# bobocode/lmono

Measured on AMD Instinct MI355X. Metric: KITTI HDL-64 scans/sec (scanRegistration + laserOdometry), higher is better.
Workload: dtype f32 features / f64 solve

## Files before the change

lmono_amd/csrc/frontend.hip:

```cpp
#include "batch.hpp"
#include "ring_decide.hpp"

namespace lmono {

__device__ __forceinline__ int ring_of(float angle, int n_lines, bool &discard)
{
    int id = 0;
    discard = false;
    if (n_lines == 16) {
        id = (int)((double)((angle + 15.0f) / 2.0f) + 0.5);
        if (id > n_lines - 1 || id < 0) discard = true;
    } else if (n_lines == 32) {
        id = (int)(((double)angle + 92.0 / 3.0) * 3.0 / 4.0);
        if (id > n_lines - 1 || id < 0) discard = true;
    } else {
        if ((double)angle >= -8.83)
            id = (int)((double)(2.0f - angle) * 3.0 + 0.5);
        else
            id = n_lines / 2 + (int)((-8.83 - (double)angle) * 2.0 + 0.5);
        if ((double)angle > 2.0 || (double)angle < -24.33 || id > 50 || id < 0) discard = true;
    }
    return id;
}

__device__ __forceinline__ bool point_valid(const float4 &p, float mr2)
{
    return isfinite(p.x) & isfinite(p.y) & isfinite(p.z) & !(p.x * p.x + p.y * p.y + p.z * p.z < mr2);
}

constexpr int kRtT = 256, kRtW = kRtT / 64;
constexpr int kRtSeg = 1024;
constexpr int kRtTile = kRtSeg * kRtW;

__device__ __forceinline__ int ring_scan_points(const BatchView &b, int s, int64_t off)
{
    const int n = (int)(b.off[s + 1] - off);
    return b.n_limit > 0 && b.n_limit < n ? b.n_limit : n;
}

__global__ __launch_bounds__(256) void k_ring_ends(BatchView b)
{
    const int s = b.scan0 + blockIdx.x;
    const int64_t off = b.off[s];
    const int n = ring_scan_points(b, s, off);
    const float4 *in = b.in + off;
    const int tid = threadIdx.x, lane = tid & 63;
    __shared__ int s_first;
    if (tid == 0) s_first = INT_MAX;
    __syncthreads();
    const float mr2 = b.min_range * b.min_range;
    for (int c0 = 0; c0 < n; c0 += 256) {
        const int i = c0 + tid;
        int lf = (i < n && point_valid(in[i], mr2)) ? i : INT_MAX;
        lf = wave_min_i(lf);
        if (lane == 0 && lf != INT_MAX) atomicMin(&s_first, lf);
        __syncthreads();
        const int f = s_first;
        __syncthreads();
        if (f != INT_MAX) break;
    }
    if (s_first == INT_MAX) {
        int *rb = b.ring_begin + s * 65;
        if (tid < 65) rb[tid] = 0;
        if (tid == 0) { b.n_cloud[s] = 0; b.scan_ends[s * 2] = -1; b.scan_ends[s * 2 + 1] = -1; b.scan_half[s] = INT_MAX; }
        return;
    }
    if (tid == 0) {
        const float4 p0 = in[s_first];
        b.scan_ori[s * 4] = (float)(-det_atan2((double)p0.y, (double)p0.x));
        float ux, uy;
        ring_start_dir(p0.x, p0.y, ux, uy);
        b.scan_ori[s * 4 + 2] = ux; b.scan_ori[s * 4 + 3] = uy;
        b.scan_ends[s * 2] = s_first; b.scan_ends[s * 2 + 1] = -1;
        b.scan_half[s] = INT_MAX;
    }
}

__global__ __launch_bounds__(kRtT) void k_ring_tag(BatchView b)
{
    const int s = b.scan0 + blockIdx.y;
    const int64_t off = b.off[s];
    const int n = ring_scan_points(b, s, off);
    const int t0 = blockIdx.x * kRtTile;
    if (t0 >= n || b.scan_ends[s * 2] < 0) return;
    const float4 *in = b.in + off;
    const int tid = threadIdx.x, lane = tid & 63, wave = tid >> 6;
    __shared__ int s_hist[kRtW][64];
    s_hist[wave][lane] = 0;
    __syncthreads();
    const float mr2 = b.min_range * b.min_range;
    const float startOri = b.scan_ori[s * 4];
    const float ux = b.scan_ori[s * 4 + 2], uy = b.scan_ori[s * 4 + 3];
    const int n_lines = b.n_lines;
    const RingMap map = ring_map(n_lines);
    int lh = INT_MAX, ll = -1;
    const int c_lo = t0 + wave * kRtSeg, c_hi = min(c_lo + kRtSeg, n);
    float4 nx[4];
#pragma unroll
    for (int q = 0; q < 4; q++) nx[q] = in[min(c_lo + 64 * q + lane, n - 1)];
    for (int r0 = c_lo; r0 < c_hi; r0 += 256) {
        float4 pq[4];
#pragma unroll
        for (int q = 0; q < 4; q++) pq[q] = nx[q];
#pragma unroll
        for (int q = 0; q < 4; q++) nx[q] = in[min(r0 + 256 + 64 * q + lane, n - 1)];
#pragma unroll
        for (int q = 0; q < 4; q++) {
            const int i = r0 + 64 * q + lane;
            const float4 p = pq[q];
            int id = -1;
            if ((i < c_hi) & point_valid(p, mr2)) {
                ll = i;
                const float q2 = p.x * p.x + p.y * p.y;
                bool past_half;
                if (!ring_half_fast(p.x, p.y, p.z, q2, __frsqrt_rn(q2) , map, ux, uy, id, past_half)) {
                    bool discard;
                    const float angle = (float)(det_atan((double)p.z / sqrt((double)(p.x * p.x + p.y * p.y))) * 180.0 / LM_PI);
                    const int r = ring_of(angle, n_lines, discard);
                    id = -1; past_half = false;
                    if (!discard) {
                        id = r;
                        float o1 = (float)(-det_atan2((double)p.y, (double)p.x));
                        if ((double)o1 < (double)startOri - LM_PI / 2.0) o1 = (float)((double)o1 + 2.0 * LM_PI);
                        else if ((double)o1 > (double)startOri + LM_PI * 3.0 / 2.0) o1 = (float)((double)o1 - 2.0 * LM_PI);
                        past_half = (double)(o1 - startOri) > LM_PI;
                    }
                }
                if (past_half) lh = min(lh, i);
            }
            if (i < c_hi) b.ring_tmp[off + i] = (int8_t)id;
            unsigned long long rem = __ballot(id >= 0);
            while (rem) {
                const int src = __ffsll((long long)rem) - 1;
                const int k = __shfl(id, src);
                const unsigned long long m = __ballot(id == k);
                if (lane == src) s_hist[wave][k] += __popcll(m);
                rem &= ~m;
            }
        }
    }
    lh = wave_min_i(lh); ll = wave_max_i(ll);
    if (lane == 0 && lh != INT_MAX) atomicMin(&b.scan_half[s], lh);
    if (lane == 0 && ll >= 0) atomicMax(&b.scan_ends[s * 2 + 1], ll);
    __syncthreads();
    if (c_lo < n) b.seg_hist[((size_t)(off >> 10) + (size_t)s + (size_t)(c_lo >> 10)) * 64 + lane] = s_hist[wave][lane];
}

__global__ __launch_bounds__(64) void k_ring_offsets(BatchView b)
{
    const int s = b.scan0 + blockIdx.x;
    if (b.scan_ends[s * 2] < 0) return;
    const int64_t off = b.off[s];
    const int n = ring_scan_points(b, s, off);
    const int nseg = (n + kRtSeg - 1) / kRtSeg, r = threadIdx.x;
// ... 184 lines not shown
            if (mh == 0u) break;
            const unsigned long long who = __ballot(ch == mh);
            unsigned int lo;
            if ((who & (who - 1ull)) == 0ull) lo = (unsigned int)__builtin_amdgcn_readlane((int)cl, __ffsll((long long)who) - 1);
            else lo = wave_max_u32_uniform(ch == mh ? cl : 0u);
            const int pind = (int)(lo >> 8), lf = (int)(lo & 15u), lb = (int)((lo >> 4) & 15u);
            largest++;
            if (largest > 20) break;
            if (lane == 0) { sel_sh[j * 20 + largest - 1] = rbeg + pind; label[pind] = largest <= 2 ? 2 : 1; }
            if (lane <= lf + lb) picked[pind - lb + lane] = 1;
            if ((unsigned int)((int)(cl >> 8) - (pind - lb)) <= (unsigned int)(lb + lf)) ch = 0u;
            {
                const int a = pind - lb - sp - lane;
                const int m0 = (a + 63) >> 6;
                if (m0 >= 0 && m0 < M && 64 * m0 <= a + lb + lf) dead |= 1u << m0;
            }
        }
    }
    while (!compact) {
        const unsigned int live = big & ~dead;
        unsigned int bh = 0u, bl = 0u;
#pragma unroll
        for (int m = 0; m < M; m++) {
            const unsigned int h = kh[m] & (unsigned int)((int)(live << (31 - m)) >> 31);
            const bool t = h >= bh;
            bh = t ? h : bh; bl = t ? kl[m] : bl;
        }
        const unsigned int mh = wave_max_u32_uniform(bh);
        if (mh == 0u) break;
        const unsigned long long who = __ballot(bh == mh);
        unsigned int lo;
        if ((who & (who - 1ull)) == 0ull) lo = (unsigned int)__builtin_amdgcn_readlane((int)bl, __ffsll((long long)who) - 1);
        else lo = wave_max_u32_uniform(bh == mh ? bl : 0u);
        const int pind = (int)(lo >> 8), lf = (int)(lo & 15u), lb = (int)((lo >> 4) & 15u);
        largest++;
        if (largest > 20) break;
        if (lane == 0) { sel_sh[j * 20 + largest - 1] = rbeg + pind; label[pind] = largest <= 2 ? 2 : 1; }
        if (lane <= lf + lb) picked[pind - lb + lane] = 1;
        {
            const int a = pind - lb - sp - lane;
            const int m0 = (a + 63) >> 6;
            if (m0 >= 0 && m0 < M && 64 * m0 <= a + lb + lf) dead |= 1u << m0;
        }
    }
    if (lane == 0) sel_sh_n[j] = largest > 20 ? 20 : largest;
    int smallest = 0;
    while (true) {
        const unsigned int live = small & ~dead;
        unsigned int bh = ~0u, bl = ~0u;
#pragma unroll
        for (int m = 0; m < M; m++) {
            const unsigned int h = kh[m] | ~(unsigned int)((int)(live << (31 - m)) >> 31);
            const bool t = h < bh;
            bh = t ? h : bh; bl = t ? kl[m] : bl;
        }
        const unsigned int mh = wave_min_u32_uniform(bh);
        if (mh == ~0u) break;
        const unsigned long long who = __ballot(bh == mh);
        unsigned int lo;
        if ((who & (who - 1ull)) == 0ull) lo = (unsigned int)__builtin_amdgcn_readlane((int)bl, __ffsll((long long)who) - 1);
        else lo = wave_min_u32_uniform(bh == mh ? bl : ~0u);
        const int pind = (int)(lo >> 8), lf = (int)(lo & 15u), lb = (int)((lo >> 4) & 15u);
        if (lane == 0) { label[pind] = -1; sel_fl[j * 4 + smallest] = rbeg + pind; }
        smallest++;
        if (smallest >= 4) break;
        if (lane <= lf + lb) picked[pind - lb + lane] = 1;
        {
            const int a = pind - lb - sp - lane;
            const int m0 = (a + 63) >> 6;
            if (m0 >= 0 && m0 < M && 64 * m0 <= a + lb + lf) dead |= 1u << m0;
        }
    }
    if (lane == 0) sel_fl_n[j] = smallest;
}

__device__ __forceinline__ int uni(int v) { return __builtin_amdgcn_readfirstlane(v); }
__device__ __forceinline__ long long uni64(long long v)
{
    const unsigned int lo = (unsigned int)__builtin_amdgcn_readfirstlane((int)(unsigned int)v), hi = (unsigned int)__builtin_amdgcn_readfirstlane((int)(unsigned int)((unsigned long long)v >> 32));
    return (long long)(((unsigned long long)hi << 32) | lo);
}
template <typename T> __device__ __forceinline__ T *uni_ptr(T *p)
{
    typedef __attribute__((address_space(1))) T GT;
    return (T *)(GT *)uni64((long long)p);
}

__host__ __device__ constexpr int sel_slice_bytes(int cap) { return 2 * cap; }

__device__ __forceinline__ void select_ring(BatchView &b, int r, int s, int lane, unsigned char *smem_w, int cap, bool may_defer, unsigned int *scratch)
{
    r = uni(r); s = uni(s);
    const int64_t off = uni64(b.off[s]);
    const int *rb = b.ring_begin + s * 65;
    const int rbeg = uni(rb[r]), rend = uni(rb[r + 1]), len = rend - rbeg;
    const int S = rbeg + 5, E = rend - 6;
    int *sel_sh = uni_ptr(b.sel_sharp + (size_t)((s * 64 + r) * kSectors) * 20);
    int *sel_sh_n = uni_ptr(b.sel_sharp_n + (s * 64 + r) * kSectors);
    int *sel_fl = uni_ptr(b.sel_flat + (size_t)((s * 64 + r) * kSectors) * 4);
    int *sel_fl_n = uni_ptr(b.sel_flat_n + (s * 64 + r) * kSectors);
    if (E - S < 6 || len > kRingCap) {
        if (lane < kSectors) { sel_sh_n[lane] = 0; sel_fl_n[lane] = 0; }
        if (lane == 0 && len > kRingCap) atomicOr(&b.status[s], kStatusRingOverflow);
        for (int i = lane; i < len; i += 64) b.label[off + rbeg + i] = 0;
        return;
    }
    if (len > cap) {
        if (may_defer && lane == 0) b.sel_todo[1 + atomicAdd(&b.sel_todo[0], 1)] = (s << 6) | r;
        return;
    }
    unsigned char *picked = smem_w;
    signed char *label = uni_ptr((signed char *)(b.label + off + rbeg));
    const float *curv = uni_ptr(b.curv + off + rbeg);
    const int span = E - S;
    unsigned long long *gap = (unsigned long long *)(picked + cap);
    for (int i0 = 0; i0 < len + 64; i0 += 64) {
        const int i = i0 + lane;
        unsigned char g = 0;
        if (i < len) { picked[i] = 0; label[i] = 0; g = b.gap[off + rbeg + i]; }
        const unsigned long long mk = __ballot(g != 0);
        if (lane == 0) gap[i0 >> 6] = mk;
    }
    __builtin_amdgcn_wave_barrier();
    for (int j = 0; j < kSectors; j++) {
        const int sp = 5 + span * j / 6;
        const int ep = 5 + span * (j + 1) / 6 - 1;
        const int slen = ep - sp + 1;
        if (slen <= 5 * 64) select_sector<5>(lane, j, sp, slen, rbeg, curv, picked, label, gap, sel_sh, sel_sh_n, sel_fl, sel_fl_n, scratch);
        else if (slen <= 6 * 64) select_sector<6>(lane, j, sp, slen, rbeg, curv, picked, label, gap, sel_sh, sel_sh_n, sel_fl, sel_fl_n, scratch);
        else select_sector<kSelMaxPerLane>(lane, j, sp, slen, rbeg, curv, picked, label, gap, sel_sh, sel_sh_n, sel_fl, sel_fl_n, scratch);
    }
}

constexpr int kSelSmallCap = 2304, kSelBigGrid = 128;

__global__ __launch_bounds__(256, 8) void k_select(BatchView b, int cap, int from_list)
{
    const int lane = threadIdx.x & 63, wave = __builtin_amdgcn_readfirstlane((int)(threadIdx.x >> 6));
    extern __shared__ __align__(16) unsigned char smem[];
    unsigned char *smem_w = smem + wave * sel_slice_bytes(cap);
    unsigned int *scratch = (unsigned int *)(smem + 4 * sel_slice_bytes(cap) + wave * kSelScratch);
    if (!from_list) {
        select_ring(b, blockIdx.x * 4 + wave, b.scan0 + blockIdx.y, lane, smem_w, cap, true, scratch);
    } else {
        const int n_todo = b.sel_todo[0];
        for (int k = blockIdx.x * 4 + wave; k < n_todo; k += gridDim.x * 4) {
            const int e = b.sel_todo[1 + k];
            select_ring(b, e & 63, e >> 6, lane, smem_w, cap, false, scratch);
        }
    }
}

constexpr int kVoxBucketSegsBig = 1024;
constexpr int kVoxSmallSlots = 9, kVoxSmallBits = 10;
constexpr int kVoxBigSlots = kRingCap / 256, kVoxBigBits = 12;
constexpr int kVoxBigGrid = 512;
template <int kSlots, int kBits, bool kSmall>
struct VoxCfg {
    static constexpr int kSegCap = kSmall ? 256 * kSlots : kVoxBucketSegsBig;
    static constexpr int kHistBytes = (1 << kBits) * 4 > kSegCap * 2 ? (1 << kBits) * 4 : kSegCap * 2;
    static constexpr int kKeyBytes = kSmall ? kSegCap * 4 + kSegCap * 2 + kSegCap * 2 + kHistBytes : kRingCap * 8;
    static constexpr int kLds = kKeyBytes + 1024 + kSlots * 4 * 8 + kSlots * 4 * 4;
};
constexpr int kVoxLdsSmall = VoxCfg<kVoxSmallSlots, kVoxSmallBits, true>::kLds;
constexpr int kVoxLdsBig = VoxCfg<kVoxBigSlots, kVoxBigBits, false>::kLds;
static_assert(2 * kVoxBucketSegsBig * 8 + (1 << kVoxBigBits) * 4 <= kRingCap * 8, "bucket sort scratch must fit the key region");
#ifdef LMONO_VOX_PROF
#define VT(i) { if (blockIdx.x == 20 && blockIdx.y == 3 && threadIdx.x == 0) vt[i] = clock64(); }
#else
#define VT(i)
#endif

__device__ __forceinline__ float wave_min_f(float v)
{
#pragma unroll
    for (int o = 32; o > 0; o >>= 1) v = fminf(v, __shfl_xor(v, o));
    return v;
}
__device__ __forceinline__ float wave_max_f(float v)
{
#pragma unroll
    for (int o = 32; o > 0; o >>= 1) v = fmaxf(v, __shfl_xor(v, o));
    return v;
}

template <int kVoxSlots, int kVoxBucketBits, bool kSmall>
__device__ __forceinline__ void voxel_ring(BatchView &b, int r, int s);

template <int kVoxSlots, int kVoxBucketBits, bool kSmall>
__global__ __launch_bounds__(256) void k_voxel(BatchView b)
{
    if (kSmall) voxel_ring<kVoxSlots, kVoxBucketBits, kSmall>(b, blockIdx.x, b.scan0 + blockIdx.y);
    else {
        const int n_todo = b.vox_todo[0];
        for (int k = blockIdx.x; k < n_todo; k += gridDim.x) {
            const int e = b.vox_todo[1 + k];
            voxel_ring<kVoxSlots, kVoxBucketBits, kSmall>(b, e & 63, e >> 6);
            __syncthreads();
        }
    }
}

template <int kVoxSlots, int kVoxBucketBits, bool kSmall>
__device__ __forceinline__ void voxel_ring(BatchView &b, int r, int s)
{
    constexpr int kVoxBuckets = 1 << kVoxBucketBits;
    constexpr int kCap = 256 * kVoxSlots;
    constexpr int kKeyBytes = VoxCfg<kVoxSlots, kVoxBucketBits, kSmall>::kKeyBytes;
    constexpr int kVoxBucketSegs = VoxCfg<kVoxSlots, kVoxBucketBits, kSmall>::kSegCap;
    const int tid = threadIdx.x, lane = tid & 63, wave = tid >> 6;
    const int64_t off = b.off[s];
#ifdef LMONO_VOX_PROF
    long long vt[8];
#endif
    VT(0)
    const int *rb = b.ring_begin + s * 65;
    const int rbeg = rb[r], rend = rb[r + 1], len = rend - rbeg;
    const int S = rbeg + 5, E = rend - 6;
    if (kSmall && len > kCap && len <= kRingCap && E - S >= 6) {
        if (tid == 0) b.vox_todo[1 + atomicAdd(&b.vox_todo[0], 1)] = (s << 6) | r;
        return;
    }
    if (E - S < 6 || len > kRingCap) {
        if (tid == 0) b.lf_n[s * 64 + r] = 0;
        return;
    }
    extern __shared__ __align__(16) unsigned char smem[];
    unsigned long long *keys = (unsigned long long *)smem;
    int *scr = (int *)(smem + kKeyBytes);
    unsigned long long *contw = (unsigned long long *)(smem + kKeyBytes + 1024);
    unsigned int *lastc = (unsigned int *)(contw + kVoxSlots * 4);
    const signed char *label = (const signed char *)(b.label + off + rbeg);
    const float4 *cl = b.cloud + off + rbeg;
    const int c_lo = 5, c_hi = len - 7;
    float mnx = FLT_MAX, mny = FLT_MAX, mnz = FLT_MAX, mxx = -FLT_MAX, mxy = -FLT_MAX, mxz = -FLT_MAX;
    int ncand = 0;
    float4 pr[kVoxSlots];
    unsigned int cand_mask = 0;
    {
        signed char lbs[kVoxSlots];
#pragma unroll
        for (int m = 0; m < kVoxSlots; m++) {
            const int i = tid + 256 * m, ic = i < len ? i : len - 1;
            lbs[m] = label[ic]; pr[m] = cl[ic];
        }
#pragma unroll
        for (int m = 0; m < kVoxSlots; m++) {
            const int i = tid + 256 * m;
            if (i >= len) pr[m] = make_float4(0.f, 0.f, 0.f, 0.f);
            if (i >= c_lo && i <= c_hi && i < len && lbs[m] <= 0) cand_mask |= 1u << m;
        }
    }
#pragma unroll
    for (int m = 0; m < kVoxSlots; m++) {
        if ((cand_mask >> m) & 1u) {
            const float4 p = pr[m];
            mnx = fminf(mnx, p.x); mny = fminf(mny, p.y); mnz = fminf(mnz, p.z);
            mxx = fmaxf(mxx, p.x); mxy = fmaxf(mxy, p.y); mxz = fmaxf(mxz, p.z);
            ncand++;
        }
    }
    VT(1)
    float *fs = (float *)scr;
    mnx = wave_min_f(mnx); mny = wave_min_f(mny); mnz = wave_min_f(mnz);
    mxx = wave_max_f(mxx); mxy = wave_max_f(mxy); mxz = wave_max_f(mxz);
    ncand = wave_sum_i(ncand);
    if (lane == 0) {
        fs[wave * 6 + 0] = mnx; fs[wave * 6 + 1] = mny; fs[wave * 6 + 2] = mnz;
        fs[wave * 6 + 3] = mxx; fs[wave * 6 + 4] = mxy; fs[wave * 6 + 5] = mxz;
        scr[32 + wave] = ncand;
    }
    __syncthreads();
    ncand = scr[32] + scr[33] + scr[34] + scr[35];
    if (ncand == 0) {
        if (tid == 0) b.lf_n[s * 64 + r] = 0;
        return;
    }
    mnx = fminf(fminf(fs[0], fs[6]), fminf(fs[12], fs[18]));
    mny = fminf(fminf(fs[1], fs[7]), fminf(fs[13], fs[19]));
    mnz = fminf(fminf(fs[2], fs[8]), fminf(fs[14], fs[20]));
    mxx = fmaxf(fmaxf(fs[3], fs[9]), fmaxf(fs[15], fs[21]));
    mxy = fmaxf(fmaxf(fs[4], fs[10]), fmaxf(fs[16], fs[22]));
    mxz = fmaxf(fmaxf(fs[5], fs[11]), fmaxf(fs[17], fs[23]));
    const float inv_leaf = 5.0f;
    const int minb0 = (int)floorf(mnx * inv_leaf), minb1 = (int)floorf(mny * inv_leaf), minb2 = (int)floorf(mnz * inv_leaf);
    const int div0 = (int)floorf(mxx * inv_leaf) - minb0 + 1, div1 = (int)floorf(mxy * inv_leaf) - minb1 + 1;
    const int mul1 = div0, mul2 = div0 * div1;
    const unsigned long long ncell = (unsigned long long)div0 * (unsigned long long)div1 * (unsigned long long)((int)floorf(mxz * inv_leaf) - minb2 + 1);
    const int cell_bits = ncell > 1ull ? 64 - __clzll((long long)(ncell - 1ull)) : 0;
    const int bshift = cell_bits > kVoxBucketBits ? cell_bits - kVoxBucketBits : 0;
    unsigned int cellr[kVoxSlots];
#pragma unroll
    for (int m = 0; m < kVoxSlots; m++) {
        unsigned int cell = ~0u;
        if ((cand_mask >> m) & 1u) {
            const float4 p = pr[m];
            const int i0 = (int)(floorf(p.x * inv_leaf) - (float)minb0);
            const int i1 = (int)(floorf(p.y * inv_leaf) - (float)minb1);
            const int i2 = (int)(floorf(p.z * inv_leaf) - (float)minb2);
            cell = (unsigned int)(i0 + i1 * mul1 + i2 * mul2);
        }
        cellr[m] = cell;
        if (lane == 63) lastc[m * 4 + wave] = cell;
    }
    unsigned long long *tmp = keys + kVoxBucketSegs;
    unsigned int *cellt = (unsigned int *)keys;
    unsigned short *idxt = (unsigned short *)((unsigned char *)keys + kVoxBucketSegs * 4);
    unsigned short *pos = (unsigned short *)((unsigned char *)keys + kVoxBucketSegs * 6);
    int *hist = kSmall ? (int *)((unsigned char *)keys + kVoxBucketSegs * 8) : (int *)(keys + 2 * kVoxBucketSegs);
    auto skey = [&](int t) -> unsigned long long {
        if (kSmall) { const int q = pos[t]; return ((unsigned long long)cellt[q] << 32) | idxt[q]; }
        return keys[t];
    };
    __syncthreads();
    VT(2)
    unsigned int head_mask = 0;
#pragma unroll
    for (int m = 0; m < kVoxSlots; m++) {
        const int i = tid + 256 * m;
        unsigned int prev = (unsigned int)__shfl_up((int)cellr[m], 1);
        if (lane == 0) prev = wave > 0 ? lastc[m * 4 + wave - 1] : (m > 0 ? lastc[(m - 1) * 4 + 3] : ~0u);
        const bool cand = cellr[m] != ~0u;
        const bool cont = cand && i > 0 && prev == cellr[m];
        const bool head = cand && !cont;
        const unsigned long long hm = __ballot(head), cm = __ballot(cont);
        if (lane == 0) { contw[m * 4 + wave] = cm; scr[64 + m * 4 + wave] = __popcll(hm); }
        if (head) head_mask |= 1u << m;
    }
    __syncthreads();
    int nseg = 0;
    int hbase[kVoxSlots];
#pragma unroll
    for (int m = 0; m < kVoxSlots; m++) {
#pragma unroll
        for (int w = 0; w < 4; w++) {
            const int c = scr[64 + m * 4 + w];
            if (w == wave) hbase[m] = nseg;
            nseg += c;
        }
    }
    int np2 = next_pow2(nseg);
    if (np2 < 2) np2 = 2;
    const bool bucket_path = nseg <= kVoxBucketSegs && ncell <= 0xffffffffull;
    if (kSmall && !bucket_path) {
        if (tid == 0) b.vox_todo[1 + atomicAdd(&b.vox_todo[0], 1)] = (s << 6) | r;
        return;
    }
    if (bucket_path) {
        for (int i = tid; i < kVoxBuckets; i += 256) hist[i] = 0;
        __syncthreads();
#pragma unroll
        for (int m = 0; m < kVoxSlots; m++)
            if ((head_mask >> m) & 1u) atomicAdd(&hist[cellr[m] >> bshift], 1);
        __syncthreads();
        VT(3)
        constexpr int kPer = kVoxBuckets / 256;
        int c[kPer], sum = 0;
#pragma unroll
        for (int q = 0; q < kPer; q++) { c[q] = hist[tid * kPer + q]; sum += c[q]; }
        const int incl_b = wave_scan_incl(sum);
        if (lane == 63) scr[44 + wave] = incl_b;
        __syncthreads();
        int run = incl_b - sum;
        for (int w = 0; w < wave; w++) run += scr[44 + w];
#pragma unroll
        for (int q = 0; q < kPer; q++) { hist[tid * kPer + q] = run; run += c[q]; }
        __syncthreads();
#pragma unroll
        for (int m = 0; m < kVoxSlots; m++)
            if ((head_mask >> m) & 1u)
            {
                const int q = atomicAdd(&hist[cellr[m] >> bshift], 1);
                if (kSmall) { cellt[q] = cellr[m]; idxt[q] = (unsigned short)(tid + 256 * m); }
                else tmp[q] = ((unsigned long long)cellr[m] << 32) | (unsigned int)(tid + 256 * m);
            }
        __syncthreads();
        for (int t = tid; t < nseg; t += 256) {
            const unsigned long long k = kSmall ? (((unsigned long long)cellt[t] << 32) | idxt[t]) : tmp[t];
            const int bk = (int)((unsigned int)(k >> 32) >> bshift);
            const int lo = bk > 0 ? hist[bk - 1] : 0, hi = hist[bk];
            int less = 0;
            for (int u = lo; u < hi; u++) less += (kSmall ? (((unsigned long long)cellt[u] << 32) | idxt[u]) : tmp[u]) < k ? 1 : 0;
            if (kSmall) pos[lo + less] = (unsigned short)t; else keys[lo + less] = k;
        }
        __syncthreads();
    } else if (!kSmall) {
#pragma unroll
        for (int m = 0; m < kVoxSlots; m++) {
            const unsigned long long hm = __ballot((head_mask >> m) & 1u);
            if ((head_mask >> m) & 1u)
                keys[hbase[m] + __popcll(hm & ((1ull << lane) - 1ull))] = ((unsigned long long)cellr[m] << 32) | (unsigned int)(tid + 256 * m);
        }
        for (int k = nseg + tid; k < np2; k += 256) keys[k] = ~0ull;
        __syncthreads();
        VT(3)
        bitonic_sort_u64(keys, np2);
    }
    VT(4)
    int *vstart = bucket_path && !kSmall ? (int *)(keys + kVoxBucketSegs) : nullptr;
    unsigned short *vstart16 = (unsigned short *)hist;
    constexpr int kRounds = (kVoxBucketSegs + 255) / 256;
    int n_out = 0, obase[kRounds];
    {
        const int rounds = (nseg + 255) / 256;
        for (int j = 0; j < rounds; j++) {
            const int t = tid + 256 * j;
            const bool st = t < nseg && (t == 0 || (unsigned int)(skey(t) >> 32) != (unsigned int)(skey(t - 1) >> 32));
            const unsigned long long sm = __ballot(st);
            if (lane == 0) scr[128 + ((j * 4 + wave) & 127)] = __popcll(sm);
        }
    }
    __syncthreads();
    float4 *outp = b.lf_tmp + off + rbeg;
    VT(5)
    if (bucket_path) {
        const int rounds = (nseg + 255) / 256;
        int total = 0;
#pragma unroll
        for (int j = 0; j < kRounds; j++)
            for (int w = 0; w < 4; w++) { if (j < rounds) { if (w == wave) obase[j] = total; total += scr[128 + j * 4 + w]; } }
        n_out = total;
#pragma unroll
        for (int j = 0; j < kRounds; j++) {
            if (j >= rounds) break;
            const int t = tid + 256 * j;
            const bool st = t < nseg && (t == 0 || (unsigned int)(skey(t) >> 32) != (unsigned int)(skey(t - 1) >> 32));
            const unsigned long long sm = __ballot(st);
            if (st) { const int o = obase[j] + __popcll(sm & ((1ull << lane) - 1ull)); if (kSmall) vstart16[o] = (unsigned short)t; else vstart[o] = t; }
        }
        __syncthreads();
        for (int v = tid; v < n_out; v += 256) {
            const int t = kSmall ? (int)vstart16[v] : vstart[v];
            const unsigned int c = (unsigned int)(skey(t) >> 32);
            float sx = 0.f, sy = 0.f, sz = 0.f, si = 0.f;
            int cnt = 0;
            for (int u = t; u < nseg; u++) {
                const unsigned long long ku = skey(u);
                if ((unsigned int)(ku >> 32) != c) break;
                const int i0 = (int)(ku & 0xffffffffull);
                int rl = 1;
                while (i0 + rl < len && ((contw[(i0 + rl) >> 6] >> ((i0 + rl) & 63)) & 1ull)) rl++;
                for (int b4 = 0; b4 < rl; b4 += 4) {
                    float4 q4[4];
#pragma unroll
                    for (int k = 0; k < 4; k++) q4[k] = b4 + k < rl ? cl[i0 + b4 + k] : make_float4(0.f, 0.f, 0.f, 0.f);
#pragma unroll
                    for (int k = 0; k < 4; k++) if (b4 + k < rl) { sx += q4[k].x; sy += q4[k].y; sz += q4[k].z; si += q4[k].w; }
                }
                cnt += rl;
            }
            const float fc = (float)cnt;
            outp[v] = make_float4(sx / fc, sy / fc, sz / fc, si / fc);
        }
    } else if (!kSmall) {
        const int chunk2 = (np2 + 255) / 256;
        const int t_lo = tid * chunk2, t_hi = min(t_lo + chunk2, nseg);
        int nstart = 0;
        for (int t = t_lo; t < t_hi; t++) {
            const unsigned int c = (unsigned int)(keys[t] >> 32);
            if (t == 0 || c != (unsigned int)(keys[t - 1] >> 32)) nstart++;
        }
        const int incl = wave_scan_incl(nstart);
        __syncthreads();
        if (lane == 63) scr[48 + wave] = incl;
        __syncthreads();
        int base = incl - nstart;
        for (int w = 0; w < wave; w++) base += scr[48 + w];
        n_out = scr[48] + scr[49] + scr[50] + scr[51];
        int o = base;
        for (int t = t_lo; t < t_hi; t++) {
            const unsigned int c = (unsigned int)(keys[t] >> 32);
            if (t == 0 || c != (unsigned int)(keys[t - 1] >> 32)) {
                float sx = 0.f, sy = 0.f, sz = 0.f, si = 0.f;
                int cnt = 0;
                for (int u = t; u < nseg && (unsigned int)(keys[u] >> 32) == c; u++) {
                    const int i0 = (int)(keys[u] & 0xffffffffull);
                    int rl = 1;
                    while (i0 + rl < len && ((contw[(i0 + rl) >> 6] >> ((i0 + rl) & 63)) & 1ull)) rl++;
                    for (int b4 = 0; b4 < rl; b4 += 4) {
                        float4 q4[4];
#pragma unroll
                        for (int k = 0; k < 4; k++) q4[k] = b4 + k < rl ? cl[i0 + b4 + k] : make_float4(0.f, 0.f, 0.f, 0.f);
#pragma unroll
                        for (int k = 0; k < 4; k++) if (b4 + k < rl) { sx += q4[k].x; sy += q4[k].y; sz += q4[k].z; si += q4[k].w; }
                    }
                    cnt += rl;
                }
                const float fc = (float)cnt;
                outp[o++] = make_float4(sx / fc, sy / fc, sz / fc, si / fc);
            }
        }
    }
    VT(6)
#ifdef LMONO_VOX_PROF
    if (blockIdx.x == 20 && blockIdx.y == 3 && tid == 0) printf("VOX len %d nseg %d nout %d | load %lld bbox+cell %lld heads %lld sort %lld runs %lld accum %lld\n", len, nseg, n_out, vt[1]-vt[0], vt[2]-vt[1], vt[3]-vt[2], vt[4]-vt[3], vt[5]-vt[4], vt[6]-vt[5]);
#endif
    if (tid == 0) b.lf_n[s * 64 + r] = n_out;
}


struct CompactIndexFeed {
    const BatchView &b;
    LiLds L;
    int s;
    bool on;
    __device__ __forceinline__ void reset(int cld, int n)
    {
        on = n <= 65535;
        if (on) li_reset<true>(L);
        else if (threadIdx.x == 0) b.li_todo[1 + atomicAdd(&b.li_todo[0], 1)] = s * 2 + cld;
    }
    __device__ __forceinline__ void point(bool ok, const float4 &p) { if (on) li_count<true>(L, ok, p.x, p.y, p.z, p.w); }
    __device__ __forceinline__ void finish(int cld, int n)
    {
        if (!on) return;
        __syncthreads();
        li_tables<true>(b, L, s, cld != 0, n);
        __builtin_amdgcn_fence(__ATOMIC_RELEASE, "workgroup");
        __syncthreads();
        __builtin_amdgcn_fence(__ATOMIC_ACQUIRE, "workgroup");
        li_scatter<true>(b, L, s, cld != 0, n);
    }
};

__device__ __forceinline__ void compact_scan(const BatchView &b, int s, CompactIndexFeed &feed)
{
    constexpr int kT = kLiT;
    const int tid = threadIdx.x;
    const int64_t off = b.off[s];
    constexpr int NE = kMaxRings * kSectors;
    __shared__ int pre_sh[NE + 1], pre_ls[NE + 1], pre_fl[NE + 1], pre_lf[kMaxRings + 1];
    const int *nsh = b.sel_sharp_n + s * NE;
    const int *nfl = b.sel_flat_n + s * NE;
    {
        const int lane = tid & 63, wave = tid >> 6;
        constexpr int kPer = NE / 64;
        int c[kPer], sum = 0;
        if (wave < 4) {
        const int *srcp = wave <= 1 ? nsh : (wave == 2 ? nfl : b.lf_n + s * 64);
#pragma unroll
        for (int q = 0; q < kPer; q++) {
            const int e = lane * kPer + q;
            const bool on = wave < 3 || e < kMaxRings;
            c[q] = srcp[on ? e : 0];
            if (!on) c[q] = 0;
        }
#pragma unroll
        for (int q = 0; q < kPer; q++) {
            if (wave == 0) c[q] = min(c[q], 2);
            sum += c[q];
        }
        const int incl = wave_scan_incl(sum);
        int run = incl - sum;
        int *dst = wave == 0 ? pre_sh : (wave == 1 ? pre_ls : (wave == 2 ? pre_fl : pre_lf));
        const int n_e = wave == 3 ? kMaxRings : NE;
#pragma unroll
        for (int q = 0; q < kPer; q++) {
            const int e = lane * kPer + q;
            if (e < n_e) dst[e] = run;
            run += c[q];
        }
        if (lane == 63) dst[n_e] = run;
        }
    }
    __syncthreads();
    const float4 *cl = b.cloud + off;
    float4 *sharp = b.sharp + (size_t)s * kMaxSharp;
    float4 *ls = b.less_sharp + (size_t)s * kMaxLessSharp;
    float4 *flat = b.flat + (size_t)s * kMaxFlat;
    float4 *lf = b.less_flat + off;
    const int *ssel = b.sel_sharp + (size_t)s * NE * 20;
    const int *fsel = b.sel_flat + (size_t)s * NE * 4;
    __shared__ int s_first[2][66], s_last[2][66], s_flag[2], s_rb[kMaxRings + 1];
    if (tid < 66) { s_first[0][tid] = INT_MAX; s_last[0][tid] = -1; s_first[1][tid] = INT_MAX; s_last[1][tid] = -1; }
    if (tid < 2) s_flag[tid] = 0;
    if (tid >= 128 && tid < 128 + kMaxRings + 1) s_rb[tid - 128] = b.ring_begin[s * 65 + tid - 128];
    const int n_ls = pre_ls[NE], n_lf = pre_lf[kMaxRings];
    feed.reset(0, n_ls);
    __syncthreads();
    static_assert(NE * 20 % 64 == 0, "feed.point() needs whole waves");
    for (int x0 = tid; x0 < NE * 20; x0 += 4 * kT) {
        int pos[4], idx[4];
#pragma unroll
        for (int q = 0; q < 4; q++) {
            const int x = x0 + kT * q, e = x / 20, k = x % 20;
            pos[q] = (x < NE * 20 && k < pre_ls[e + 1] - pre_ls[e]) ? pre_ls[e] + k : -1;
        }
#pragma unroll
        for (int q = 0; q < 4; q++) idx[q] = ssel[pos[q] >= 0 ? x0 + kT * q : 0];
        float4 p4[4];
#pragma unroll
        for (int q = 0; q < 4; q++) { const float4 *src = pos[q] >= 0 ? cl + idx[q] : b.cloud; p4[q] = *src; }
#pragma unroll
        for (int q = 0; q < 4; q++) {
            const float4 p = p4[q];
            if (pos[q] >= 0) {
                const int x = x0 + kT * q, e = x / 20, k = x % 20;
                ls[pos[q]] = p;
                if (k < 2) sharp[pre_sh[e] + k] = p;
                int v = (int)p.w;
                v = v < 0 ? 0 : (v > 65 ? 65 : v);
                atomicMin(&s_first[0][v], pos[q]);
                atomicMax(&s_last[0][v], pos[q]);
            }
            feed.point(pos[q] >= 0, p);
        }
    }
    for (int x0 = tid; x0 < NE * 4; x0 += 2 * kT) {
        int pos[2], idx[2];
#pragma unroll
        for (int q = 0; q < 2; q++) {
            const int x = x0 + kT * q, e = x / 4, k = x % 4;
            pos[q] = (x < NE * 4 && k < pre_fl[e + 1] - pre_fl[e]) ? pre_fl[e] + k : -1;
        }
#pragma unroll
        for (int q = 0; q < 2; q++) idx[q] = fsel[pos[q] >= 0 ? x0 + kT * q : 0];
        float4 p2[2];
#pragma unroll
        for (int q = 0; q < 2; q++) { const float4 *src = pos[q] >= 0 ? cl + idx[q] : b.cloud; p2[q] = *src; }
#pragma unroll
        for (int q = 0; q < 2; q++) if (pos[q] >= 0) flat[pos[q]] = p2[q];
    }
    feed.finish(0, n_ls);
    __syncthreads();
    feed.reset(1, n_lf);
    __syncthreads();
    for (int base = 0; base < n_lf; base += 4 * kT) {
        const int j0 = base + tid;
        float4 v4[4];
#pragma unroll
        for (int q = 0; q < 4; q++) {
            const int j = j0 + kT * q;
            v4[q] = make_float4(0.f, 0.f, 0.f, 0.f);
            if (j < n_lf) {
                int lo = 0, hi = kMaxRings;
                while (hi - lo > 1) { const int mid = (lo + hi) >> 1; if (pre_lf[mid] <= j) lo = mid; else hi = mid; }
                v4[q] = b.lf_tmp[off + s_rb[lo] + (j - pre_lf[lo])];
            }
        }
// ... 46 lines not shown
```

Measured before the change: 128,500.

## Rework small voxel bucket sort with packed 16-bit counters and DPP scans

Reworks the small-ring voxel downsampling sort. Bucket counters are now packed 16-bit values, two per word, giving twice as many buckets in the same LDS. Keys are packed 32-bit words with the 12-bit index folded in, and the rank pass also computes cell-start flags so later passes need no indirect key compares. Shuffle-based wave min/max/scan reductions become DPP sequences with readlane, per-wave base offsets come from a single wave scan instead of serial loops, and run-length search over the continuity bitmask uses ctz over 64-bit windows. The changes rely on new static bounds (ring index under 4096 and the ncell limit) and on two padding words in the continuity array.

```diff
diff --git a/lmono_amd/csrc/frontend.hip b/lmono_amd/csrc/frontend.hip
--- a/lmono_amd/csrc/frontend.hip
+++ b/lmono_amd/csrc/frontend.hip
@@ -1,5 +1,6 @@
 #include "batch.hpp"
 #include "ring_decide.hpp"
+#include "vox_runs.hpp"
 
 namespace lmono {
 
@@ -490,16 +491,18 @@
 }
 
 constexpr int kVoxBucketSegsBig = 1024;
-constexpr int kVoxSmallSlots = 9, kVoxSmallBits = 10;
+constexpr int kVoxSmallSlots = 9, kVoxSmallBits = 11;
 constexpr int kVoxBigSlots = kRingCap / 256, kVoxBigBits = 12;
 constexpr int kVoxBigGrid = 512;
 template <int kSlots, int kBits, bool kSmall>
 struct VoxCfg {
     static constexpr int kSegCap = kSmall ? 256 * kSlots : kVoxBucketSegsBig;
-    static constexpr int kHistBytes = (1 << kBits) * 4 > kSegCap * 2 ? (1 << kBits) * 4 : kSegCap * 2;
+    static constexpr int kHistBytes = (1 << kBits) * 2 > kSegCap * 2 ? (1 << kBits) * 2 : kSegCap * 2;
     static constexpr int kKeyBytes = kSmall ? kSegCap * 4 + kSegCap * 2 + kSegCap * 2 + kHistBytes : kRingCap * 8;
-    static constexpr int kLds = kKeyBytes + 1024 + kSlots * 4 * 8 + kSlots * 4 * 4;
+    static constexpr int kLds = kKeyBytes + 1024 + (kSlots * 4 + 2) * 8 + kSlots * 4 * 4;
 };
+static_assert(256 * kVoxSmallSlots <= 4096, "a first index of the small instantiation has 12 bits");
+static_assert((1 << kVoxSmallBits) == 2048, "the small instantiation's counters are one uint4 per thread");
 constexpr int kVoxLdsSmall = VoxCfg<kVoxSmallSlots, kVoxSmallBits, true>::kLds;
 constexpr int kVoxLdsBig = VoxCfg<kVoxBigSlots, kVoxBigBits, false>::kLds;
 static_assert(2 * kVoxBucketSegsBig * 8 + (1 << kVoxBigBits) * 4 <= kRingCap * 8, "bucket sort scratch must fit the key region");
@@ -509,16 +512,39 @@
 #define VT(i)
 #endif
 
+template <int kCtrl, int kRowMask>
+__device__ __forceinline__ float dpp_mov_f32(float v, float ident)
+{
+    return __uint_as_float(dpp_mov_u32<kCtrl, kRowMask>(__float_as_uint(v), __float_as_uint(ident)));
+}
 __device__ __forceinline__ float wave_min_f(float v)
 {
-#pragma unroll
-    for (int o = 32; o > 0; o >>= 1) v = fminf(v, __shfl_xor(v, o));
-    return v;
+    v = fminf(v, dpp_mov_f32<0x111, 0xf>(v, FLT_MAX));
+    v = fminf(v, dpp_mov_f32<0x112, 0xf>(v, FLT_MAX));
+    v = fminf(v, dpp_mov_f32<0x114, 0xf>(v, FLT_MAX));
+    v = fminf(v, dpp_mov_f32<0x118, 0xf>(v, FLT_MAX));
+    v = fminf(v, dpp_mov_f32<0x142, 0xa>(v, FLT_MAX));
+    v = fminf(v, dpp_mov_f32<0x143, 0xc>(v, FLT_MAX));
+    return __uint_as_float((unsigned int)__builtin_amdgcn_readlane((int)__float_as_uint(v), 63));
 }
 __device__ __forceinline__ float wave_max_f(float v)
 {
-#pragma unroll
-    for (int o = 32; o > 0; o >>= 1) v = fmaxf(v, __shfl_xor(v, o));
+    v = fmaxf(v, dpp_mov_f32<0x111, 0xf>(v, -FLT_MAX));
+    v = fmaxf(v, dpp_mov_f32<0x112, 0xf>(v, -FLT_MAX));
+    v = fmaxf(v, dpp_mov_f32<0x114, 0xf>(v, -FLT_MAX));
+    v = fmaxf(v, dpp_mov_f32<0x118, 0xf>(v, -FLT_MAX));
+    v = fmaxf(v, dpp_mov_f32<0x142, 0xa>(v, -FLT_MAX));
+    v = fmaxf(v, dpp_mov_f32<0x143, 0xc>(v, -FLT_MAX));
+    return __uint_as_float((unsigned int)__builtin_amdgcn_readlane((int)__float_as_uint(v), 63));
+}
+__device__ __forceinline__ int wave_scan_incl_dpp(int v)
+{
+    v += (int)dpp_mov_u32<0x111, 0xf>((unsigned int)v, 0u);
+    v += (int)dpp_mov_u32<0x112, 0xf>((unsigned int)v, 0u);
+    v += (int)dpp_mov_u32<0x114, 0xf>((unsigned int)v, 0u);
+    v += (int)dpp_mov_u32<0x118, 0xf>((unsigned int)v, 0u);
+    v += (int)dpp_mov_u32<0x142, 0xa>((unsigned int)v, 0u);
+    v += (int)dpp_mov_u32<0x143, 0xc>((unsigned int)v, 0u);
     return v;
 }
 
@@ -567,7 +593,7 @@
     unsigned long long *keys = (unsigned long long *)smem;
     int *scr = (int *)(smem + kKeyBytes);
     unsigned long long *contw = (unsigned long long *)(smem + kKeyBytes + 1024);
-    unsigned int *lastc = (unsigned int *)(contw + kVoxSlots * 4);
+    unsigned int *lastc = (unsigned int *)(contw + kVoxSlots * 4 + 2);
     const signed char *label = (const signed char *)(b.label + off + rbeg);
     const float4 *cl = b.cloud + off + rbeg;
     const int c_lo = 5, c_hi = len - 7;
@@ -642,14 +668,10 @@
         if (lane == 63) lastc[m * 4 + wave] = cell;
     }
     unsigned long long *tmp = keys + kVoxBucketSegs;
-    unsigned int *cellt = (unsigned int *)keys;
-    unsigned short *idxt = (unsigned short *)((unsigned char *)keys + kVoxBucketSegs * 4);
-    unsigned short *pos = (unsigned short *)((unsigned char *)keys + kVoxBucketSegs * 6);
+    unsigned int *wsc = (unsigned int *)keys;
+    unsigned short *bkt = (unsigned short *)((unsigned char *)keys + kVoxBucketSegs * 4);
+    unsigned short *srt = (unsigned short *)((unsigned char *)keys + kVoxBucketSegs * 6);
     int *hist = kSmall ? (int *)((unsigned char *)keys + kVoxBucketSegs * 8) : (int *)(keys + 2 * kVoxBucketSegs);
-    auto skey = [&](int t) -> unsigned long long {
-        if (kSmall) { const int q = pos[t]; return ((unsigned long long)cellt[q] << 32) | idxt[q]; }
-        return keys[t];
-    };
     __syncthreads();
     VT(2)
     unsigned int head_mask = 0;
@@ -665,26 +687,69 @@
         if (lane == 0) { contw[m * 4 + wave] = cm; scr[64 + m * 4 + wave] = __popcll(hm); }
         if (head) head_mask |= 1u << m;
     }
-    __syncthreads();
-    int nseg = 0;
+    if (tid < 2) contw[kVoxSlots * 4 + tid] = 0ull;
+    __syncthreads();
+    const int wave_u = __builtin_amdgcn_readfirstlane(wave);
+    const int hc = lane < kVoxSlots * 4 ? scr[64 + lane] : 0;
+    const int hincl = wave_scan_incl_dpp(hc);
+    const int nseg = __builtin_amdgcn_readlane(hincl, 63);
     int hbase[kVoxSlots];
-#pragma unroll
-    for (int m = 0; m < kVoxSlots; m++) {
-#pragma unroll
-        for (int w = 0; w < 4; w++) {
-            const int c = scr[64 + m * 4 + w];
-            if (w == wave) hbase[m] = nseg;
-            nseg += c;
-        }
+    if (!kSmall) {
+#pragma unroll
+        for (int m = 0; m < kVoxSlots; m++) hbase[m] = __builtin_amdgcn_readlane(hincl - hc, m * 4 + wave_u);
     }
     int np2 = next_pow2(nseg);
     if (np2 < 2) np2 = 2;
-    const bool bucket_path = nseg <= kVoxBucketSegs && ncell <= 0xffffffffull;
+    const bool bucket_path = nseg <= kVoxBucketSegs && ncell <= (kSmall ? 0x80000000ull : 0xffffffffull);
     if (kSmall && !bucket_path) {
         if (tid == 0) b.vox_todo[1 + atomicAdd(&b.vox_todo[0], 1)] = (s << 6) | r;
         return;
     }
-    if (bucket_path) {
+    if (bucket_path && kSmall) {
+        uint4 *hw4 = (uint4 *)hist;
+        unsigned int *hw = (unsigned int *)hist;
+        const unsigned short *h16 = (const unsigned short *)hist;
+        hw4[tid] = make_uint4(0u, 0u, 0u, 0u);
+        __syncthreads();
+#pragma unroll
+        for (int m = 0; m < kVoxSlots; m++)
+            if ((head_mask >> m) & 1u) { const unsigned int bk = cellr[m] >> bshift; atomicAdd(&hw[bk >> 1], 1u << ((bk & 1u) * 16u)); }
+        __syncthreads();
+        VT(3)
+        const uint4 cw = hw4[tid];
+        const unsigned int c0 = cw.x & 0xffffu, c1 = cw.x >> 16, c2 = cw.y & 0xffffu, c3 = cw.y >> 16;
+        const unsigned int c4 = cw.z & 0xffffu, c5 = cw.z >> 16, c6 = cw.w & 0xffffu, c7 = cw.w >> 16;
+        const int sum = (int)(c0 + c1 + c2 + c3 + c4 + c5 + c6 + c7);
+        const int incl_b = wave_scan_incl_dpp(sum);
+        if (lane == 63) scr[44 + wave] = incl_b;
+        __syncthreads();
+        unsigned int run = (unsigned int)(incl_b - sum);
+        for (int w = 0; w < wave; w++) run += (unsigned int)scr[44 + w];
+        uint4 ew;
+        { const unsigned int e0 = run, e1 = e0 + c0, e2 = e1 + c1, e3 = e2 + c2, e4 = e3 + c3, e5 = e4 + c4, e6 = e5 + c5, e7 = e6 + c6;
+          ew = make_uint4(e0 | (e1 << 16), e2 | (e3 << 16), e4 | (e5 << 16), e6 | (e7 << 16)); }
+        hw4[tid] = ew;
+        __syncthreads();
+        const unsigned int cmask = (1u << bshift) - 1u;
+#pragma unroll
+        for (int m = 0; m < kVoxSlots; m++)
+            if ((head_mask >> m) & 1u) {
+                const unsigned int bk = cellr[m] >> bshift, sh = (bk & 1u) * 16u;
+                const unsigned int q = (atomicAdd(&hw[bk >> 1], 1u << sh) >> sh) & 0xffffu;
+                wsc[q] = ((cellr[m] & cmask) << 12) | (unsigned int)(tid + 256 * m);
+                bkt[q] = (unsigned short)bk;
+            }
+        __syncthreads();
+        for (int t = tid; t < nseg; t += 256) {
+            const unsigned int k = wsc[t], kc = k & ~0xfffu;
+            const int bk = bkt[t];
+            const int lo = bk > 0 ? h16[bk - 1] : 0, hi = h16[bk];
+            int less = 0, lessc = 0;
+            for (int u = lo; u < hi; u++) { const unsigned int ku = wsc[u]; less += ku < k ? 1 : 0; lessc += ku < kc ? 1 : 0; }
+            srt[lo + less] = (unsigned short)((k & 0xfffu) | (less == lessc ? 0x8000u : 0u));
+        }
+        __syncthreads();
+    } else if (!kSmall && bucket_path) {
         for (int i = tid; i < kVoxBuckets; i += 256) hist[i] = 0;
         __syncthreads();
 #pragma unroll
@@ -696,7 +761,7 @@
         int c[kPer], sum = 0;
 #pragma unroll
         for (int q = 0; q < kPer; q++) { c[q] = hist[tid * kPer + q]; sum += c[q]; }
-        const int incl_b = wave_scan_incl(sum);
+        const int incl_b = wave_scan_incl_dpp(sum);
         if (lane == 63) scr[44 + wave] = incl_b;
         __syncthreads();
         int run = incl_b - sum;
@@ -706,20 +771,18 @@
         __syncthreads();
 #pragma unroll
         for (int m = 0; m < kVoxSlots; m++)
-            if ((head_mask >> m) & 1u)
-            {
+            if ((head_mask >> m) & 1u) {
                 const int q = atomicAdd(&hist[cellr[m] >> bshift], 1);
-                if (kSmall) { cellt[q] = cellr[m]; idxt[q] = (unsigned short)(tid + 256 * m); }
-                else tmp[q] = ((unsigned long long)cellr[m] << 32) | (unsigned int)(tid + 256 * m);
+                tmp[q] = ((unsigned long long)cellr[m] << 32) | (unsigned int)(tid + 256 * m);
             }
         __syncthreads();
         for (int t = tid; t < nseg; t += 256) {
-            const unsigned long long k = kSmall ? (((unsigned long long)cellt[t] << 32) | idxt[t]) : tmp[t];
+            const unsigned long long k = tmp[t];
             const int bk = (int)((unsigned int)(k >> 32) >> bshift);
             const int lo = bk > 0 ? hist[bk - 1] : 0, hi = hist[bk];
             int less = 0;
-            for (int u = lo; u < hi; u++) less += (kSmall ? (((unsigned long long)cellt[u] << 32) | idxt[u]) : tmp[u]) < k ? 1 : 0;
-            if (kSmall) pos[lo + less] = (unsigned short)t; else keys[lo + less] = k;
+            for (int u = lo; u < hi; u++) less += tmp[u] < k ? 1 : 0;
+            keys[lo + less] = k;
         }
         __syncthreads();
     } else if (!kSmall) {
@@ -738,54 +801,57 @@
     int *vstart = bucket_path && !kSmall ? (int *)(keys + kVoxBucketSegs) : nullptr;
     unsigned short *vstart16 = (unsigned short *)hist;
     constexpr int kRounds = (kVoxBucketSegs + 255) / 256;
-    int n_out = 0, obase[kRounds];
-    {
-        const int rounds = (nseg + 255) / 256;
+    const int rounds = (nseg + 255) / 256;
+    int n_out = 0;
+    unsigned int st_mask = 0;
+    if (bucket_path) {
         for (int j = 0; j < rounds; j++) {
             const int t = tid + 256 * j;
-            const bool st = t < nseg && (t == 0 || (unsigned int)(skey(t) >> 32) != (unsigned int)(skey(t - 1) >> 32));
+            bool st;
+            if (kSmall) st = t < nseg && (srt[t] & 0x8000u) != 0u;
+            else st = t < nseg && (t == 0 || (unsigned int)(keys[t] >> 32) != (unsigned int)(keys[t - 1] >> 32));
             const unsigned long long sm = __ballot(st);
-            if (lane == 0) scr[128 + ((j * 4 + wave) & 127)] = __popcll(sm);
+            if (lane == 0) scr[128 + j * 4 + wave] = __popcll(sm);
+            if (st) st_mask |= 1u << j;
         }
     }
     __syncthreads();
     float4 *outp = b.lf_tmp + off + rbeg;
+    auto add_run = [&](int i0, float &sx, float &sy, float &sz, float &si, int &cnt) {
+        const int rl = vox_run_length(contw, i0);
+        for (int b4 = 0; b4 < rl; b4 += 4) {
+            float4 q4[4];
+#pragma unroll
+            for (int k = 0; k < 4; k++) q4[k] = b4 + k < rl ? cl[i0 + b4 + k] : make_float4(0.f, 0.f, 0.f, 0.f);
+#pragma unroll
+            for (int k = 0; k < 4; k++) if (b4 + k < rl) { sx += q4[k].x; sy += q4[k].y; sz += q4[k].z; si += q4[k].w; }
+        }
+        cnt += rl;
+    };
     VT(5)
     if (bucket_path) {
-        const int rounds = (nseg + 255) / 256;
-        int total = 0;
-#pragma unroll
-        for (int j = 0; j < kRounds; j++)
-            for (int w = 0; w < 4; w++) { if (j < rounds) { if (w == wave) obase[j] = total; total += scr[128 + j * 4 + w]; } }
-        n_out = total;
+        const int oc = lane < rounds * 4 ? scr[128 + lane] : 0;
+        const int oincl = wave_scan_incl_dpp(oc);
+        n_out = __builtin_amdgcn_readlane(oincl, 63);
 #pragma unroll
         for (int j = 0; j < kRounds; j++) {
             if (j >= rounds) break;
             const int t = tid + 256 * j;
-            const bool st = t < nseg && (t == 0 || (unsigned int)(skey(t) >> 32) != (unsigned int)(skey(t - 1) >> 32));
+            const bool st = (st_mask >> j) & 1u;
+            const int obase = __builtin_amdgcn_readlane(oincl - oc, j * 4 + wave_u);
             const unsigned long long sm = __ballot(st);
-            if (st) { const int o = obase[j] + __popcll(sm & ((1ull << lane) - 1ull)); if (kSmall) vstart16[o] = (unsigned short)t; else vstart[o] = t; }
+            if (st) { const int o = obase + __popcll(sm & ((1ull << lane) - 1ull)); if (kSmall) vstart16[o] = (unsigned short)t; else vstart[o] = t; }
         }
         __syncthreads();
         for (int v = tid; v < n_out; v += 256) {
-            const int t = kSmall ? (int)vstart16[v] : vstart[v];
-            const unsigned int c = (unsigned int)(skey(t) >> 32);
+            int t0, t1;
+            if (kSmall) { t0 = vstart16[v]; t1 = v + 1 < n_out ? (int)vstart16[v + 1] : nseg; }
+            else { t0 = vstart[v]; t1 = v + 1 < n_out ? vstart[v + 1] : nseg; }
             float sx = 0.f, sy = 0.f, sz = 0.f, si = 0.f;
             int cnt = 0;
-            for (int u = t; u < nseg; u++) {
-                const unsigned long long ku = skey(u);
-                if ((unsigned int)(ku >> 32) != c) break;
-                const int i0 = (int)(ku & 0xffffffffull);
-                int rl = 1;
-                while (i0 + rl < len && ((contw[(i0 + rl) >> 6] >> ((i0 + rl) & 63)) & 1ull)) rl++;
-                for (int b4 = 0; b4 < rl; b4 += 4) {
-                    float4 q4[4];
-#pragma unroll
-                    for (int k = 0; k < 4; k++) q4[k] = b4 + k < rl ? cl[i0 + b4 + k] : make_float4(0.f, 0.f, 0.f, 0.f);
-#pragma unroll
-                    for (int k = 0; k < 4; k++) if (b4 + k < rl) { sx += q4[k].x; sy += q4[k].y; sz += q4[k].z; si += q4[k].w; }
-                }
-                cnt += rl;
+            for (int u = t0; u < t1; u++) {
+                const int i0 = kSmall ? (int)(srt[u] & 0xfffu) : (int)(keys[u] & 0xffffffffull);
+                add_run(i0, sx, sy, sz, si, cnt);
             }
             const float fc = (float)cnt;
             outp[v] = make_float4(sx / fc, sy / fc, sz / fc, si / fc);
@@ -812,17 +878,7 @@
                 float sx = 0.f, sy = 0.f, sz = 0.f, si = 0.f;
                 int cnt = 0;
                 for (int u = t; u < nseg && (unsigned int)(keys[u] >> 32) == c; u++) {
-                    const int i0 = (int)(keys[u] & 0xffffffffull);
-                    int rl = 1;
-                    while (i0 + rl < len && ((contw[(i0 + rl) >> 6] >> ((i0 + rl) & 63)) & 1ull)) rl++;
-                    for (int b4 = 0; b4 < rl; b4 += 4) {
-                        float4 q4[4];
-#pragma unroll
-                        for (int k = 0; k < 4; k++) q4[k] = b4 + k < rl ? cl[i0 + b4 + k] : make_float4(0.f, 0.f, 0.f, 0.f);
-#pragma unroll
-                        for (int k = 0; k < 4; k++) if (b4 + k < rl) { sx += q4[k].x; sy += q4[k].y; sz += q4[k].z; si += q4[k].w; }
-                    }
-                    cnt += rl;
+                    add_run((int)(keys[u] & 0xffffffffull), sx, sy, sz, si, cnt);
                 }
                 const float fc = (float)cnt;
                 outp[o++] = make_float4(sx / fc, sy / fc, sz / fc, si / fc);
diff --git a/lmono_amd/csrc/vox_runs.hpp b/lmono_amd/csrc/vox_runs.hpp
--- /dev/null
+++ b/lmono_amd/csrc/vox_runs.hpp
@@ -0,0 +1,33 @@
+#pragma once
+
+#if defined(__HIPCC__)
+#define LMONO_VOX_HD __host__ __device__ __forceinline__
+#else
+#define LMONO_VOX_HD inline
+#endif
+
+LMONO_VOX_HD int vox_trailing_ones(unsigned long long w)
+{
+    const unsigned long long z = ~w;
+    return z ? __builtin_ctzll(z) : 64;
+}
+
+LMONO_VOX_HD unsigned long long vox_window(const unsigned long long *bits, int p)
+{
+    const int w = p >> 6, sh = p & 63;
+    const unsigned long long a = bits[w], b = bits[w + 1];
+    return sh ? (a >> sh) | (b << (64 - sh)) : a;
+}
+
+LMONO_VOX_HD int vox_run_length(const unsigned long long *contw, int i0)
+{
+    int p = i0 + 1;
+    int n = vox_trailing_ones(vox_window(contw, p));
+    int rl = 1 + n;
+    while (n == 64) {
+        p += 64;
+        n = vox_trailing_ones(vox_window(contw, p));
+        rl += n;
+    }
+    return rl;
+}
```

New measurement: 131,300 (median of 6 runs). 1.02x the previous value.
